# shunpeizhang/nebula

Measured on AMD Instinct MI355X. Metric: GO 3 STEPS traversed edges/sec (TEPS) at 1/2/4/8 GPU; FIND SHORTEST PATH p50, higher is better.
Workload: dtype int64; 1 GPU; GO 3 STEPS FROM <root> OVER e WHERE e.w < 50 YIELD e._dst, 16 single-root queries per step; graph=RMAT-26, parts=100, roots=16, queries_in_flight=6, parallelism=single, vertices_rank0=32799492, live_edges_out_plus_in_rank0=2120776948

## Files before the change

nebula_amd/csrc/final.hip:

```cpp
#include <hip/hip_runtime.h>

#include "nbg_internal.h"

namespace nbg {
namespace {

constexpr int FB = 256;
constexpr int FW = FB / 64;
constexpr int FV = VT;
static_assert(FV == 4 && TILE == 256, "the head mask is 4 words of 64 tile positions");

__device__ __forceinline__ void wave_lds_sync() {
  __builtin_amdgcn_fence(__ATOMIC_RELEASE, "wavefront");
  __builtin_amdgcn_wave_barrier();
  __builtin_amdgcn_fence(__ATOMIC_ACQUIRE, "wavefront");
}

template <typename T>
__device__ __forceinline__ T ld(const T* p) {
  return __hip_atomic_load(p, __ATOMIC_RELAXED, __HIP_MEMORY_SCOPE_WAVEFRONT);
}

template <int WB>
struct WType { using T = int64_t; };
template <> struct WType<1> { using T = int8_t; };
template <> struct WType<2> { using T = int16_t; };
template <> struct WType<4> { using T = int32_t; };

}

template <int WB, bool ONE>
__global__ void __launch_bounds__(FB) __attribute__((amdgpu_waves_per_eu(8)))
k_final_dst(FinalDstArgs a) {
  __shared__ unsigned long long sMaskAll[FW][FV];
  __shared__ uint32_t sDeltaAll[FW][TILE + 1];
  __shared__ unsigned long long sBase;
  const int lane = threadIdx.x & 63;
  const int w = __builtin_amdgcn_readfirstlane(threadIdx.x >> 6);
  unsigned long long* const sMask = sMaskAll[w];
  uint32_t* const sDelta = sDeltaAll[w];
  const uint64_t g = (uint64_t)gridDim.x * FW;
  uint64_t t = (uint64_t)blockIdx.x * FW + w;
  const __attribute__((address_space(4))) uint32_t* const tsplit =
      (const __attribute__((address_space(4))) uint32_t*)a.tsplit;
  const uint64_t tmax = a.tsplit_n ? a.tsplit_n - 1 : 0;
  auto clampt = [&](uint64_t x) { return x < tmax ? x : tmax; };
  const uint32_t sp0 = tsplit[clampt(t)], sp1 = tsplit[clampt(t + 1)];
  const uint32_t sq0 = tsplit[clampt(t + g)], sq1 = tsplit[clampt(t + g + 1)];
// ... 25 lines not shown
    *st = q == 0 ? 0u : (q - 1 < n32 ? x0 : 0xFFFFFFFFu);
    *en = q < n32 ? x1 : 0xFFFFFFFFu;
    *r = q < n32 ? rr : 0u;
  };
  const typename WType<WB>::T* const wcol = static_cast<const typename WType<WB>::T*>(a.wcol);
  int64_t wlo = a.lo, whi = a.hi;
  bool wneg = a.where_neg != 0;
  if (wlo < INT32_MIN) wlo = INT32_MIN;
  if (whi > INT32_MAX) whi = INT32_MAX;
  if (wlo > whi) {
    wlo = INT32_MIN;
    whi = INT32_MAX;
    wneg = !wneg;
  }
  const uint32_t wbase = (uint32_t)(int32_t)wlo, wspan = (uint32_t)(whi - wlo);
  auto store_rows = [&](const int64_t (&dv)[FV], uint32_t pm, uint64_t region) {
    uint32_t off = 0;
#pragma unroll
    for (int i = 0; i < FV; ++i) {
      const bool pass = (pm >> i) & 1u;
      const unsigned long long bal = __ballot(pass);
      const uint64_t row = region + off + __builtin_amdgcn_mbcnt_hi((uint32_t)(bal >> 32),
                                                                  __builtin_amdgcn_mbcnt_lo((uint32_t)bal, 0u));
      off += (uint32_t)__popcll(bal);
      if constexpr (ONE) {
        if (pass) a.out[0][row] = dv[i];
      } else {
        for (int y = 0; y < a.nyields; ++y)
          if (pass) a.out[y][row] = ((a.const_mask >> y) & 1u) ? a.yconst[y] : dv[i];
      }
    }
  };
  int64_t pdv[FV];
  uint32_t ppm = 0;
  uint64_t preg = 0;
#pragma unroll
  for (int i = 0; i < FV; ++i) pdv[i] = 0;
  uint64_t a0 = 0, a1 = 0, n0 = 0, n1 = 0;
  uint32_t e_pre = 0, f_pre = 0, r_pre = 0;
  if (t < ntiles) {
    a0 = sp0;
    a1 = (t + 1) * TILE >= npath ? n : sp1;
    if (t + g < ntiles) {
      n0 = sq0;
      n1 = (t + g + 1) * TILE >= npath ? n : sq1;
    }
    stage(a0, &e_pre, &f_pre, &r_pre);
  }
// ... 33 lines not shown
      }
    }
    wave_lds_sync();
    uint32_t jj[FV];
    {
      uint32_t before = 0;
#pragma unroll
      for (int i = 0; i < FV; ++i) {
        const unsigned long long m = sMask[i];
        const uint32_t c = before + (uint32_t)__popcll(m & le);
        before += (uint32_t)__popcll(m);
        jj[i] = b0 + (uint32_t)(i * 64 + lane) + sDelta[c];
      }
    }
    wave_lds_sync();
    int64_t dv[FV];
    typename WType<WB>::T x[FV];
    {
      const uint32_t jsafe = nb > 0 ? (uint32_t)__builtin_amdgcn_readfirstlane((int)jj[0]) : 0u;
#pragma unroll
      for (int i = 0; i < FV; ++i)
        if (i * 64 + lane >= nb) jj[i] = jsafe;
#pragma unroll
      for (int i = 0; i < FV; ++i) dv[i] = ld(a.dst_vid + jj[i]);
      if constexpr (WB != 0) {
#pragma unroll
        for (int i = 0; i < FV; ++i) x[i] = ld(wcol + jj[i]);
      }
    }
    store_rows(pdv, ppm, preg);
    uint32_t pm = 0;
#pragma unroll
    for (int i = 0; i < FV; ++i) {
      const bool act = i * 64 + lane < nb;
      bool pass = act;
      if constexpr (WB == 8) {
        const int64_t v = (int64_t)x[i];
        pass = act & (((v >= a.lo) & (v <= a.hi)) != (a.where_neg != 0));
      } else if constexpr (WB != 0) {
// ... 27 lines not shown
  }
  __syncthreads();
  if (threadIdx.x == 0) a.blk_rows[blockIdx.x] = (uint32_t)sBase;
}

namespace {

template <int WB>
void launch_wb(const FinalDstArgs& a, bool one, unsigned grid, hipStream_t s) {
  if (one) hipLaunchKernelGGL((k_final_dst<WB, true>), dim3(grid), dim3(FB), 0, s, a);
  else hipLaunchKernelGGL((k_final_dst<WB, false>), dim3(grid), dim3(FB), 0, s, a);
}

}

hipError_t launch_final_dst(const FinalDstArgs& a, int wbytes, bool one, unsigned grid, hipStream_t s) {
  switch (wbytes) {
    case 0: launch_wb<0>(a, one, grid, s); break;
    case 1: launch_wb<1>(a, one, grid, s); break;
    case 2: launch_wb<2>(a, one, grid, s); break;
    case 4: launch_wb<4>(a, one, grid, s); break;
    case 8: launch_wb<8>(a, one, grid, s); break;
    default: return hipErrorInvalidValue;
  }
  return hipGetLastError();
}

}
```

nebula_amd/csrc/finalcopy.hip:

```cpp
#include <hip/hip_runtime.h>

#include "nbg_internal.h"

namespace nbg {
namespace {

constexpr int CB = 256;
constexpr int CW = CB / 64;
constexpr int CH = 512;
constexpr int CM = CH / 64;
constexpr int CI = CH / 128;
static_assert(CH % 128 == 0, "a chunk is whole 16-byte stores of 64 lanes");

typedef long long row2 __attribute__((ext_vector_type(2), aligned(8)));

__device__ __forceinline__ void wave_lds_sync() {
  __builtin_amdgcn_fence(__ATOMIC_RELEASE, "wavefront");
  __builtin_amdgcn_wave_barrier();
  __builtin_amdgcn_fence(__ATOMIC_ACQUIRE, "wavefront");
}

template <typename T>
__device__ __forceinline__ T ld(const T* p) {
  return __hip_atomic_load(p, __ATOMIC_RELAXED, __HIP_MEMORY_SCOPE_WAVEFRONT);
}

__device__ __forceinline__ uint32_t lanes_below(unsigned long long b) {
  return __builtin_amdgcn_mbcnt_hi((uint32_t)(b >> 32), __builtin_amdgcn_mbcnt_lo((uint32_t)b, 0u));
}

}

__global__ void __launch_bounds__(CB) __attribute__((amdgpu_waves_per_eu(8)))
k_final_copy(FinalCopyArgs a) {
  __shared__ unsigned long long sMaskAll[CW][CM];
  __shared__ uint32_t sDeltaAll[CW][CH + 1];
  const int lane = threadIdx.x & 63;
  const int w = __builtin_amdgcn_readfirstlane(threadIdx.x >> 6);
  unsigned long long* const sMask = sMaskAll[w];
  uint32_t* const sDelta = sDeltaAll[w];
  const uint32_t g = gridDim.x * CW;
  const uint32_t t_first = blockIdx.x * CW + w;
  const unsigned long long packed = *a.acc;
  const uint64_t n = packed >> 32;
  const uint32_t n32 = (uint32_t)n, total = (uint32_t)packed;
  if (blockIdx.x == 0 && threadIdx.x == 0) {
    if (a.stat_e && !a.full_rp) *a.stat_e += total;
    if (a.stat_n) *a.stat_n = n;
  }
// ... 86 lines not shown
      idx[2 * i] = r0 + p + sDelta[base + (uint32_t)__popcll(m & le0)];
      idx[2 * i + 1] = r0 + p + 1 + sDelta[base + (uint32_t)__popcll(m & le1)];
      before += c0 + (uint32_t)__popcll(m1);
    }
    wave_lds_sync();
    const uint32_t jsafe = ok ? (uint32_t)__builtin_amdgcn_readfirstlane((int)idx[0]) : 0u;
#pragma unroll
    for (int i = 0; i < CI; ++i) {
      const uint32_t p = (uint32_t)(i * 128 + 2 * lane);
      if (!ok || p >= nb) idx[2 * i] = jsafe;
      if (!ok || p + 1 >= nb) idx[2 * i + 1] = jsafe;
    }
    return ok;
  };
  auto store2 = [&](int64_t* p, row2 v) { __builtin_nontemporal_store(v, reinterpret_cast<row2*>(p)); };
  auto store_chunk = [&](const row2 (&v)[CI], uint32_t tt) {
    int64_t* const o = out + (uint64_t)tt * CH + 2 * lane;
#pragma unroll
    for (int i = 0; i < CI; ++i) store2(o + i * 128, v[i]);
  };
  auto fetch = [&](uint32_t tt, uint32_t kb, uint32_t x0, uint32_t x1, uint32_t rr, row2 (&v)[CI]) {
    const uint32_t r0 = tt * CH;
    uint32_t st, en, rs;
    window(kb, x0, x1, rr, &st, &en, &rs);
    const unsigned long long own = __ballot(kb + (uint32_t)lane < n32 && st <= r0 && r0 < en);
    const int l0 = own ? __ffsll((long long)own) - 1 : 0;
    const uint32_t st0 = (uint32_t)__builtin_amdgcn_readlane((int)st, l0);
    const uint32_t en0 = (uint32_t)__builtin_amdgcn_readlane((int)en, l0);
    const uint32_t rs0 = (uint32_t)__builtin_amdgcn_readlane((int)rs, l0);
    if (own && en0 - r0 >= (uint32_t)CH) {
      const int64_t* const src = a.dst_vid + (uint64_t)(rs0 + (r0 - st0)) + 2 * lane;
#pragma unroll
      for (int i = 0; i < CI; ++i) v[i] = *reinterpret_cast<const row2*>(src + i * 128);
    } else {
      uint32_t idx[2 * CI];
      const bool ok = resolve(kb, r0, CH, st, en, rs, idx);
      if (!ok && lane == 0) atomicOr(a.err_flag, SPLIT_BAD);
#pragma unroll
      for (int i = 0; i < CI; ++i) {
        v[i].x = ld(a.dst_vid + idx[2 * i]);
        v[i].y = ld(a.dst_vid + idx[2 * i + 1]);
      }
    }
  };
  const uint32_t mine = t_first < nfull ? (nfull - 1 - t_first) / g + 1 : 0u;
  uint32_t a_lo = 0, a_hi = 0, a_step = 0, a_val = 0, b_lo = 0, b_hi = 0, b_step = 0, b_val = 0;
  bool a_pend = false, b_pend = false;
  uint32_t s_kb = 0, s_x0 = 0, s_x1 = 0, s_rr = 0;
  row2 cur[CI];
#pragma unroll
  for (int i = 0; i < CI; ++i) cur[i] = row2{0, 0};
  for (uint32_t it = 0; mine && it < mine + 4; ++it) {
    if (it >= 4) store_chunk(cur, t_first + (it - 4) * g);
    if (it >= 3 && it < mine + 3) fetch(t_first + (it - 3) * g, s_kb, s_x0, s_x1, s_rr, cur);
    if (it >= 2 && it < mine + 2) {
      if (b_pend) narrow(&b_lo, &b_hi, b_step, b_val, (t_first + (it - 2) * g) * CH);
      s_kb = b_lo;
      stage(s_kb, &s_x0, &s_x1, &s_rr);
    }
    if (it >= 1 && it < mine + 1) {
      b_lo = a_lo;
      b_hi = a_hi;
      if (a_pend) narrow(&b_lo, &b_hi, a_step, a_val, (t_first + (it - 1) * g) * CH);
      b_pend = b_hi - b_lo > 64;
      if (b_pend) {
        b_step = (b_hi - b_lo + 63) / 64;
// ... 6 lines not shown
      if (a_pend) {
        a_step = (a_hi - a_lo + 63) / 64;
        a_val = probe(a_lo, a_hi, a_step);
      }
    }
  }
  const uint32_t rem = total - nfull * CH;
  if (rem && t_first == nfull % g) {
    const uint32_t r0 = nfull * CH;
    const uint32_t kb = bracket(r0);
    uint32_t x0, x1, rr, st, en, rs, idx[2 * CI];
    stage(kb, &x0, &x1, &rr);
    window(kb, x0, x1, rr, &st, &en, &rs);
    const bool ok = resolve(kb, r0, rem, st, en, rs, idx);
    if (!ok && lane == 0) atomicOr(a.err_flag, SPLIT_BAD);
    int64_t v[2 * CI];
#pragma unroll
    for (int i = 0; i < 2 * CI; ++i) v[i] = ld(a.dst_vid + idx[i]);
#pragma unroll
    for (int i = 0; i < CI; ++i) {
      const uint32_t p = (uint32_t)(i * 128 + 2 * lane);
      if (ok && p < rem) out[(uint64_t)r0 + p] = v[2 * i];
      if (ok && p + 1 < rem) out[(uint64_t)r0 + p + 1] = v[2 * i + 1];
    }
  }
  if (a.full_rp) {
    unsigned long long sum = 0;
    for (uint64_t i = (uint64_t)t_first * 64 + lane; i < n; i += (uint64_t)g * 64) {
      const uint32_t v = a.ids[i];
      if (v != NO_ROW && (!a.visible || a.visible[v])) sum += a.full_rp[v + 1] - a.full_rp[v];
    }
    for (int o = 32; o; o >>= 1) sum += __shfl_down(sum, o, 64);
    if (lane == 0 && sum) atomicAdd(a.stat_e, sum);
  }
  if (threadIdx.x == 0) a.blk_rows[blockIdx.x] = blockIdx.x == 0 ? total : 0u;
}

hipError_t launch_final_copy(const FinalCopyArgs& a, unsigned grid, hipStream_t s) {
  hipLaunchKernelGGL(k_final_copy, dim3(grid), dim3(CB), 0, s, a);
  return hipGetLastError();
}

}
```

nebula_amd/csrc/go.cpp:

```cpp
#include <algorithm>
#include <array>
#include <atomic>
#include <cstring>
#include <ctime>
#include <iterator>
#include <set>
#include <unordered_map>

#include "engine.h"
#include "nbg_rows.h"

using namespace nbg;

struct nbg_go_stmt {
  Engine* eng = nullptr;
  uint64_t id = 0;
  std::vector<int32_t> over;
  std::vector<TypeProgram> plist;
  int ncols = 0;
  uint32_t steps = 1;
  int32_t deferred = NBG_OK;
  std::string deferred_msg;
  std::string dst_unknown;
  bool distinct = false;
// ... 1 lines not shown
  std::vector<std::vector<uint8_t>> wclass;
  bool misaligned = false, float_col = false;
  bool derived = false;
  uint64_t sout_row_bytes = 0;
  bool uses_input = false;
  std::vector<int64_t> in_ids;
  std::vector<std::vector<int64_t>> in_cols;
  uint64_t in_n = 0;
  int64_t* d_in_ids = nullptr;
  int64_t** d_in_cols = nullptr;
  std::vector<int64_t*> d_in_col_ptrs;
  std::vector<std::string> in_xstr;
  uint32_t* d_xoff = nullptr;
  char* d_xbytes = nullptr;
  bool idx_on = false;
  double idx_after = 0.25;
  uint64_t idx_budget = UINT64_MAX;
  uint64_t final_scanned = 0;
  StmtIndex idx;
  bool idx_tried = false;
  void free_input_index() {
    for (void* p : {(void*)d_in_ids, (void*)d_in_cols, (void*)d_xoff, (void*)d_xbytes})
      if (p) (void)hipFree(p);
    for (auto* p : d_in_col_ptrs)
      if (p) (void)hipFree(p);
    d_in_ids = nullptr;
    d_in_cols = nullptr;
    d_xoff = nullptr;
    d_xbytes = nullptr;
    d_in_col_ptrs.clear();
// ... 505 lines not shown
  Engine& E = q.E;
  nbg_go_stmt* st = q.st;
  if (!st->idx_on || st->idx_tried || st->steps < 2 || E.partitioned() || st->deferred || st->over.empty()) return;
  auto it = E.snap.types.find(st->over[0]);
  if (it == E.snap.types.end()) return;
  const DevEdgeType& dt = it->second;
  if ((double)st->final_scanned < st->idx_after * (double)dt.num_edges) return;
  st->idx_tried = true;
  if ((uint64_t)q.cap < (uint64_t)std::max(dt.max_degree, 0)) return;
  const TypeProgram& prog = st->plist[0];
  if (prog.where_const) return;
  StmtIndexSpec sp{};
  if (!ws_final_where(prog, q.args_for(dt), &sp)) return;
  sp.nv = E.snap.nv;
  sp.edges = dt.num_edges;
  double ms = 0;
  const bool ok = stmtidx_build(sp, st->idx_budget, E.stream, &st->idx, &ms);
  if (getenv("NBG_STMT_INDEX_TRACE")) {
    if (ok)
      fprintf(stderr, "[stmt index] statement %llu type %d: built in %.3f ms after %llu final-step edges, %llu of %llu "
                      "edges pass, %.1f MB\n", (unsigned long long)st->id, st->over[0], ms,
              (unsigned long long)st->final_scanned, (unsigned long long)st->idx.rows,
              (unsigned long long)dt.num_edges, (double)st->idx.bytes / 1e6);
    else
      fprintf(stderr, "[stmt index] statement %llu type %d: not built (memory budget or allocation), %.3f ms\n",
              (unsigned long long)st->id, st->over[0], ms);
  }
}

static void go_workspace(GoQuery& q, const GoStarts& S, uint64_t num_starts, Workspace** wsp) {
  Engine& E = q.E;
  if (!q.lrc && *wsp) {
    const int32_t rrc = ws_release(E, wsp, q.stream);
    if (rrc) q.local_fail(rrc, E.last_error);
  }
  const uint64_t need = q.part ? std::max<uint64_t>(num_starts, 1) : S.n;
  const uint64_t e_need = std::max<uint64_t>(E.snap.max_edges(), S.start_edges);
  if (!q.lrc && (!*wsp || need > ws_cap_frontier(*wsp) || S.n + S.start_edges > ws_cap_items(*wsp))) {
// ... 152 lines not shown
      }
    }
    if (s == 1 && !final && hop1_slots) he = ws_set_hop_slots(ws, hop1_slots);
    for (size_t i = 0; he == hipSuccess && i < over.size(); ++i) {
      auto it = E.snap.types.find(over[i]);
      if (it == E.snap.types.end()) continue;
      ExpandArgs a = q.args_for(it->second);
      a.bt_first = s == 1;
      if (!final) {
        he = ws_expand_mark(ws, a, n_bound, it->second.num_edges, (int)s, (int)i, S.inline_of(i, s), np0);
      } else if (q.st->deferred || (plist[i].where_const && !plist[i].where_const_val)) {
        he = ws_scan_only(ws, a, n_bound, (int)s, (int)i);
      } else if (const StmtIndex* ix = q.index_of(i)) {
        const uint32_t* const full = a.row_ptr;
        a.row_ptr = ix->rp;
        a.dst_vid = ix->dst;
        he = ws_expand_final(ws, a, n_bound, ebound[i], (int)s, (int)i, plist[i], plan.region[i], plan.blk_cap[i],
                             nullptr, full);
      } else {
        he = ws_expand_final(ws, a, n_bound, ebound[i], (int)s, (int)i, plist[i], plan.region[i], plan.blk_cap[i],
                             S.inline_of(i, s));
      }
    }
    if (inject) he = hipErrorLaunchFailure;
    if (!final && he == hipSuccess) {
      he = q.part ? ws_exchange(ws, (int)s, np0) : ws_finish_step(ws, (int)s, np0);
      n_bound = E.snap.nv;
    }
  }
  return he;
}

static hipError_t go_end(const GoQuery& q, const RowPlan& plan, bool device) {
// ... 555 lines not shown
  for (int32_t i = 0; i < cap && i < (int32_t)req.size(); ++i) out[i] = req[i];
  return (int32_t)req.size();
}

int32_t nbg_go_prepare(nbg_engine* h, const nbg_go_request* req, nbg_go_stmt** out) {
  if (!h) return NBG_E_INVALID_ARGUMENT;
  Engine& E = h->e;
  std::lock_guard<std::mutex> lg(E.mu);
  const int32_t rc = go_prepare(E, req, out);
  if (rc || (*out)->steps < 2) return rc;
  {
    nbg_go_stmt* st = *out;
    const char* on = getenv("NBG_STMT_INDEX");
    const char* after = getenv("NBG_STMT_INDEX_AFTER");
    const char* mb = getenv("NBG_STMT_INDEX_MB");
    st->idx_on = !(on && atoi(on) == 0);
    if (after) st->idx_after = std::max(0.0, atof(after));
    if (mb) st->idx_budget = strtoull(mb, nullptr, 10) << 20;
  }
  if (hipSetDevice(E.cfg.device) != hipSuccess) return NBG_OK;
  const uint64_t rows = stmt_row_bound(E, *out);
  auto reserve = [&](Workspace* w) {
    if (w && !E.holders.count(w)) (void)ws_reserve_rows(w, rows, (*out)->ncols);
  };
  reserve(E.ws);
  for (auto& q : E.slots) reserve(q.ws);
  E.row_reserve = std::max(E.row_reserve, rows);
  E.col_reserve = std::max(E.col_reserve, (*out)->ncols);
  return NBG_OK;
}

// ... 16 lines not shown
```

nebula_amd/csrc/kernels.hip:

```cpp
#include <hip/hip_runtime.h>
#include <array>
#include <cstddef>

#include <cstdio>
#include <cstring>
#include <vector>

#include "aggops.h"
#include "stage.h"
#include "ws.h"

namespace nbg {


struct DegSrc {
  const uint32_t* row_ptr;
  const uint8_t* visible;
  uint32_t cap;
};

struct ListOut {
  uint32_t* ids;
  uint32_t* seg_end;
  uint32_t* seg_rs;
// ... 2175 lines not shown
    unsigned long long e = 0;
    for (int t = 0; t < ntypes; ++t) e += q->e_st[s][t];
    g[1 + (MAX_STEPS + 2) + s] = e;
  }
}

static double prof_bytes(const Workspace* w, const Prof::Rec& r, const QState& q) {
  switch (r.kid) {
    case K_RELIST: return 12.0 * (double)q.step_n[r.step];
    case K_EXPAND_MARK: return 4.0 * (double)q.e_st[r.step][r.tix];
    case K_COMPACT: case K_BITS_COMPACT: return 16.0 * (double)q.step_n[r.step + 1];
    case K_PACK: case K_ALLTOALL: case K_ROOTS: return r.cols;
    case K_EXPAND_FINAL: {
      double rows = 0;
      for (unsigned b = 0; b < w->final_grid[r.tix]; ++b) rows += (double)w->h_blk_rows[(size_t)r.tix * EXPAND_GRID + b];
      if (r.cols < 0) return 8.0 * rows + 8.0 * rows * r.kout + 12.0 * (double)q.step_n[r.step];
      return (double)q.e_st[r.step][r.tix] * (4.0 + 8.0 * r.cols) + 8.0 * rows * r.kout;
    }
    default: return 0.0;
  }
}
static double prof_bytes_path(const Prof::Rec& r, const PState& p) {
  const int i = r.step < PATH_REC ? r.step : PATH_REC - 1;
  switch (r.kid) {
    case K_RELIST: return 12.0 * (double)p.ln[i];
    case K_BFS: return 4.0 * (double)p.le[i];
    case K_GATHER: return 8.0 * (double)p.lc[i];
    case K_DEGSUM: return 12.0 * (double)p.ln[i];
    default: return 0.0;
  }
}
// ... 566 lines not shown
  if (prog.yield_reg.size() > (size_t)MAX_YIELDS) return false;
  const FastProg f = detect_fast(prog, a);
  if (!final_where_shape(f, a)) return false;
  sp->row_ptr = a.row_ptr;
  sp->dst_vid = a.dst_vid;
  sp->wcol = f.wcol;
  sp->wbytes = f.wbytes;
  sp->lo = f.lo;
  sp->hi = f.hi;
  sp->where_neg = f.where_neg;
  return true;
}

hipError_t ws_expand_final(Workspace* w, const ExpandArgs& a0, uint64_t n_bound, uint64_t e_bound, int step, int tix,
                           const TypeProgram& prog, uint64_t region_base, uint64_t blk_cap, const InlineList* il,
                           const uint32_t* full_row_ptr) {
  if (step > MAX_STEPS || tix >= MAX_TYPES_Q) return hipErrorInvalidValue;
  const bool inl = inline_start_list(w, tix, il);
  if (full_row_ptr && (inl || tix != 0 || !w->seg_ready)) return hipErrorInvalidValue;
  const ListRef L = inl ? ListRef{nullptr, nullptr, &w->q->step_n[step], 0} : prepare_list(w, a0, n_bound, step, tix);
  ExpandArgs a = a0;
  a.frontier = L.ids;
  a.tsplit = inl ? nullptr : set_split(w, L.set);
  uint32_t* const l_end = set_end(w, L.set);
  uint32_t* const l_rs = set_rs(w, L.set);
  FinalParams fp{};
  fp.prog = w->d_prog + (size_t)tix * MAX_PROGRAM;
  fp.where_len = prog.where_len;
  fp.where_reg = prog.where_reg;
  fp.prog_len = (int)prog.code.size();
  fp.nyields = (int)prog.yield_reg.size();
  for (int y = 0; y < fp.nyields; ++y) {
// ... 63 lines not shown
    if (full_row_ptr && one && final_copy_on()) {
      FinalCopyArgs ca{};
      ca.acc = fa.acc;
      ca.seg_end = fa.seg_end;
      ca.seg_rs = fa.seg_rs;
      ca.dst_vid = fa.dst_vid;
      ca.out = fa.out[0];
      ca.region_base = region_base;
      ca.blk_rows = fa.blk_rows;
      ca.stat_e = fa.stat_e;
      ca.stat_n = fa.stat_n;
      ca.err_flag = fa.err_flag;
      ca.full_rp = fa.full_rp;
      ca.ids = fa.ids;
      ca.visible = fa.visible;
      le = launch_final_copy(ca, grid.x, w->stream);
    } else {
      le = launch_final_dst(fa, fp.fast.has_where ? fp.fast.wbytes : 0, one, grid.x, w->stream);
    }
    if (le != hipSuccess) {
      prof_end(w, p, K_EXPAND_FINAL, step, tix, 0.0, 0.0);
      return le;
    }
  } else {
    launch(grid, lds, w->stream, a, L.acc, l_end, l_rs, w->flags, fp, BfsParams{}, e_st, L.stat_n, inl ? il : nullptr);
  }
  prof_end(w, p, K_EXPAND_FINAL, step, tix, full_row_ptr ? -1.0 : (double)edge_columns_read(prog), (double)fp.nyields);
  w->final_grid[tix] = final_grid(n_bound, e_bound);
  return hipGetLastError();
}



hipError_t ws_backtracker(Workspace* w, int64_t** out, int64_t** in) {
  if (!w->bt) HIP_TRY(hipMalloc((void**)&w->bt, (w->nv + 1) * 8));
  if (w->comm && !w->h_btc) {
    const uint64_t G = (uint64_t)w->comm->world, nwords = G * w->npad / 64;
    if (!w->bt_out) HIP_TRY(hipMalloc((void**)&w->bt_out, G * w->npad * 8));
    if (!w->bt_pack) HIP_TRY(hipMalloc((void**)&w->bt_pack, G * w->npad * 8));
    if (!w->bt_recv) HIP_TRY(hipMalloc((void**)&w->bt_recv, G * w->npad * 8));
    if (!w->bt_pre) HIP_TRY(hipMalloc((void**)&w->bt_pre, 2 * nwords * 4));
    if (!w->bt_boff) HIP_TRY(hipMalloc((void**)&w->bt_boff, 2 * (nwords / RW_BLOCK) * 4));
// ... 1583 lines not shown
```

nebula_amd/csrc/nbg_internal.h:

```cpp
#pragma once
#include <hip/hip_runtime_api.h>

#include <array>
#include <cstdint>
#include <map>
#include <memory>
#include <string>
#include <unordered_map>
#include <vector>

#include "../../include/nbg.h"

namespace nbg {

constexpr uint32_t NO_ROW = 0xFFFFFFFFu;

struct Column {
  std::string name;
  int32_t type;
};
struct Schema {
  int64_t version = 0;
  std::vector<Column> cols;
  int find(const std::string& n) const {
// ... 287 lines not shown
  uint64_t in_n;
  const int64_t* const* in_cols;
  DevStrings str;
  int64_t now_sec;
  uint64_t rand_seed;
};

struct FinalDstArgs {
  const unsigned long long* acc;
  const uint32_t* seg_end;
  const uint32_t* seg_rs;
  const uint32_t* tsplit;
  uint64_t tsplit_n;
  const int64_t* dst_vid;
  const void* wcol;
  int64_t lo, hi;
  int32_t where_neg;
  int32_t nyields;
  uint64_t const_mask;
  int64_t yconst[MAX_YIELDS];
  int64_t* out[MAX_YIELDS];
  uint64_t region_base, blk_cap;
  uint32_t* blk_rows;
  unsigned long long* stat_e;
  unsigned long long* stat_n;
  unsigned long long* err_flag;
  const uint32_t* full_rp;
  const uint32_t* ids;
  const uint8_t* visible;
};
hipError_t launch_final_dst(const FinalDstArgs& a, int wbytes, bool one, unsigned grid, hipStream_t s);

struct FinalCopyArgs {
  const unsigned long long* acc;
  const uint32_t* seg_end;
  const uint32_t* seg_rs;
  const int64_t* dst_vid;
  int64_t* out;
  uint64_t region_base;
  uint32_t* blk_rows;
  unsigned long long* stat_e;
  unsigned long long* stat_n;
  unsigned long long* err_flag;
  const uint32_t* full_rp;
  const uint32_t* ids;
  const uint8_t* visible;
};
hipError_t launch_final_copy(const FinalCopyArgs& a, unsigned grid, hipStream_t s);

struct StmtIndexSpec {
  const uint32_t* row_ptr;
  const int64_t* dst_vid;
  uint64_t nv, edges;
  const void* wcol;
  int wbytes;
  int64_t lo, hi;
  int where_neg;
};
struct StmtIndex {
  uint32_t* rp = nullptr;
  int64_t* dst = nullptr;
  uint64_t rows = 0;
  uint64_t bytes = 0;
};
bool stmtidx_build(const StmtIndexSpec& sp, uint64_t budget_bytes, hipStream_t s, StmtIndex* out, double* ms);
void stmtidx_free(StmtIndex* ix);

constexpr int LVL_BITS = 6;
constexpr uint32_t MAX_PATH_LEN = (1u << LVL_BITS) - 1;
constexpr int PSLOTS = 8;
enum PathLabel { LAB_F = 0, LAB_B = 1, LAB_S = 2, LAB_M = 3, NUM_LABS = 4 };
constexpr int GREEDY_HOP_BLOCKS = 64;
constexpr int PATH_REC = 64;

struct PState {
  unsigned long long n[PSLOTS];
  unsigned long long total;
  unsigned long long edges;
// ... 524 lines not shown
uint64_t rd_block_bytes(uint64_t len, uint64_t nchunks, uint64_t rows);
int32_t ws_rows_decode(hipStream_t stream, const uint8_t* data, uint64_t len, const uint64_t* chunk_start, uint64_t nchunks,
                       const uint32_t* row_off, uint64_t rows, void* block, const RdPlan& plan, Workspace** outw,
                       RdRecord* rec, StageProf<RD_KINDS>* prof, std::string* err);

hipError_t ws_begin_query(Workspace* w, const uint32_t* starts, uint64_t n, const std::vector<TypeProgram>* progs,
                          uint64_t stmt_id);
hipError_t ws_begin_query_resident(Workspace* w, uint64_t n, const std::vector<TypeProgram>* progs, uint64_t stmt_id);
hipError_t ws_expand_mark(Workspace* w, const ExpandArgs& a, uint64_t n_bound, uint64_t e_bound, int step, int tix,
                          const InlineList* il, const ExpandArgs* next0);
hipError_t ws_finish_step(Workspace* w, int step, const ExpandArgs* next0);
void ws_set_mark_claims(Workspace* w, bool claims);
void ws_set_wake(Workspace* w, bool flag);
hipError_t ws_expand_final(Workspace* w, const ExpandArgs& a, uint64_t n_bound, uint64_t e_bound, int step, int tix,
                           const TypeProgram& prog, uint64_t region_base, uint64_t blk_cap, const InlineList* il = nullptr,
                           const uint32_t* full_row_ptr = nullptr);
bool ws_final_where(const TypeProgram& prog, const ExpandArgs& a, StmtIndexSpec* sp);
hipError_t ws_scan_only(Workspace* w, const ExpandArgs& a, uint64_t n_bound, int step, int tix);
hipError_t ws_backtracker(Workspace* w, int64_t** out, int64_t** in);
void ws_backtracker_off(Workspace* w);
hipError_t ws_end_query(Workspace* w);
hipError_t ws_end_query_async(Workspace* w);
struct SmallPack {
  int ntypes, ncols;
  uint64_t region[MAX_TYPES_Q], blk_cap[MAX_TYPES_Q];
  uint32_t grid[MAX_TYPES_Q];
};
constexpr uint64_t SMALL_ROWS_WORDS = 32768;
hipError_t ws_end_query_async_small(Workspace* w, const SmallPack& sp);
const int64_t* ws_host_small_rows(Workspace* w, uint64_t count);
hipError_t ws_end_query_wait(Workspace* w);
// ... 90 lines not shown
```

nebula_amd/csrc/stmtidx.hip:

```cpp
#include <hip/hip_runtime.h>

#include <algorithm>
#include <chrono>
#include <cstring>
#include <rocprim/rocprim.hpp>

#include "nbg_internal.h"

namespace nbg {
namespace {

constexpr int BT = 256;

unsigned grid_for(uint64_t n) {
  const uint64_t g = (n + BT - 1) / BT;
  return (unsigned)std::min<uint64_t>(std::max<uint64_t>(g, 1), 1u << 16);
}

#define GRID_STRIDE(i, n) \
  for (uint64_t i = (uint64_t)blockIdx.x * BT + threadIdx.x; i < (n); i += (uint64_t)gridDim.x * BT)

template <typename T>
struct Pass {
  const T* col;
  int64_t lo, hi;
  bool neg;
  uint64_t n;
  __device__ __forceinline__ uint32_t operator()(uint64_t j) const {
    if (j >= n) return 0u;
    const int64_t v = (int64_t)col[j];
    return (((v >= lo) & (v <= hi)) != neg) ? 1u : 0u;
  }
};

template <typename T>
__global__ void __launch_bounds__(BT) k_idx_scatter(Pass<T> pass, const uint32_t* __restrict__ pos,
                                                    const int64_t* __restrict__ dst, int64_t* __restrict__ out) {
  GRID_STRIDE(j, pass.n)
    if (pass(j)) out[pos[j]] = dst[j];
}

__global__ void __launch_bounds__(BT) k_idx_rows(const uint32_t* __restrict__ row_ptr, const uint32_t* __restrict__ pos,
                                                 uint32_t* __restrict__ rp, uint64_t nv) {
  GRID_STRIDE(v, nv + 1) rp[v] = pos[row_ptr[v]];
}

struct Temps {
  uint32_t* pos = nullptr;
  void* scan = nullptr;
  ~Temps() {
    if (pos) (void)hipFree(pos);
    if (scan) (void)hipFree(scan);
  }
};

template <typename T>
bool build_as(const StmtIndexSpec& sp, uint64_t budget, hipStream_t s, StmtIndex* out) {
  const uint64_t E = sp.edges, nv = sp.nv;
  const Pass<T> pass{static_cast<const T*>(sp.wcol), sp.lo, sp.hi, sp.where_neg != 0, E};
  auto flags = rocprim::make_transform_iterator(rocprim::make_counting_iterator<uint64_t>(0), pass);
  size_t scan_bytes = 0;
  Temps t;
  if (rocprim::exclusive_scan(nullptr, scan_bytes, flags, t.pos, 0u, E + 1, rocprim::plus<uint32_t>(), s) != hipSuccess)
    return false;
  const uint64_t rp_bytes = (nv + 1) * 4, temp_bytes = (E + 1) * 4 + scan_bytes;
  if (rp_bytes + temp_bytes > budget) return false;
  StmtIndex ix;
  bool ok = hipMalloc((void**)&t.pos, (E + 1) * 4) == hipSuccess &&
            hipMalloc(&t.scan, std::max<size_t>(scan_bytes, 1)) == hipSuccess &&
            hipMalloc((void**)&ix.rp, rp_bytes) == hipSuccess;
  ok = ok && rocprim::exclusive_scan(t.scan, scan_bytes, flags, t.pos, 0u, E + 1, rocprim::plus<uint32_t>(), s) ==
                 hipSuccess;
  uint32_t total = 0;
  ok = ok && hipMemcpyAsync(&total, t.pos + E, 4, hipMemcpyDeviceToHost, s) == hipSuccess &&
       hipStreamSynchronize(s) == hipSuccess;
  const uint64_t dst_bytes = std::max<uint64_t>(total, 1) * 8;
  ok = ok && rp_bytes + dst_bytes + temp_bytes <= budget && hipMalloc((void**)&ix.dst, dst_bytes) == hipSuccess;
  if (ok) {
    if (!total) ok = hipMemsetAsync(ix.dst, 0, 8, s) == hipSuccess;
    hipLaunchKernelGGL(k_idx_rows, dim3(grid_for(nv + 1)), dim3(BT), 0, s, sp.row_ptr, t.pos, ix.rp, nv);
    if (total) hipLaunchKernelGGL(k_idx_scatter<T>, dim3(grid_for(E)), dim3(BT), 0, s, pass, t.pos, sp.dst_vid, ix.dst);
    ok = ok && hipGetLastError() == hipSuccess && hipStreamSynchronize(s) == hipSuccess;
  }
  if (!ok) {
    (void)hipGetLastError();
    stmtidx_free(&ix);
    return false;
  }
  ix.rows = total;
  ix.bytes = rp_bytes + dst_bytes;
  *out = ix;
  return true;
}

}

void stmtidx_free(StmtIndex* ix) {
  if (ix->rp) (void)hipFree(ix->rp);
  if (ix->dst) (void)hipFree(ix->dst);
  *ix = StmtIndex{};
}

bool stmtidx_build(const StmtIndexSpec& sp, uint64_t budget_bytes, hipStream_t s, StmtIndex* out, double* ms) {
  *out = StmtIndex{};
  if (!sp.row_ptr || !sp.dst_vid || !sp.wcol || !sp.edges || sp.edges >= 0xFFFFFFFFull) return false;
  size_t free_b = 0, total_b = 0;
  if (hipMemGetInfo(&free_b, &total_b) != hipSuccess) return false;
  const uint64_t budget = std::min<uint64_t>(budget_bytes, free_b / 2);
  if (hipStreamSynchronize(s) != hipSuccess) return false;
  const auto t0 = std::chrono::steady_clock::now();
  bool ok = false;
  switch (sp.wbytes) {
    case 1: ok = build_as<int8_t>(sp, budget, s, out); break;
    case 2: ok = build_as<int16_t>(sp, budget, s, out); break;
    case 4: ok = build_as<int32_t>(sp, budget, s, out); break;
    case 8: ok = build_as<int64_t>(sp, budget, s, out); break;
    default: break;
  }
  if (ms) *ms = std::chrono::duration<double, std::milli>(std::chrono::steady_clock::now() - t0).count();
  return ok;
}

}
```

Measured before the change: 591.1 billion TEPS.

## Store statement-index destination IDs as 32-bit offsets from a base

When building the per-statement filtered edge index, a reduction first finds the min/max destination vertex ID. If the span fits in 32 bits, destinations are stored as uint32 offsets from that base. The final-step dst and copy kernels read the narrower column and widen it back to int64 on output. This halves the bytes read from the index in the final GO step, at the cost of an extra reduction pass during index build and more kernel template variants.

```diff
diff --git a/nebula_amd/csrc/final.hip b/nebula_amd/csrc/final.hip
--- a/nebula_amd/csrc/final.hip
+++ b/nebula_amd/csrc/final.hip
@@ -27,11 +27,22 @@
 template <> struct WType<2> { using T = int16_t; };
 template <> struct WType<4> { using T = int32_t; };
 
-}
-
-template <int WB, bool ONE>
+constexpr int DST32 = -4;
+template <int WB>
+struct DType { using T = int64_t; };
+template <> struct DType<DST32> { using T = uint32_t; };
+
+}
+
+template <int WBX, bool ONE>
 __global__ void __launch_bounds__(FB) __attribute__((amdgpu_waves_per_eu(8)))
 k_final_dst(FinalDstArgs a) {
+  constexpr int WB = WBX == DST32 ? 0 : WBX;
+  using DT = typename DType<WBX>::T;
+  auto wide = [&](DT c) -> int64_t {
+    if constexpr (WBX == DST32) return (int64_t)((uint64_t)a.dst_base + (uint64_t)c);
+    else return c;
+  };
   __shared__ unsigned long long sMaskAll[FW][FV];
   __shared__ uint32_t sDeltaAll[FW][TILE + 1];
   __shared__ unsigned long long sBase;
@@ -87,7 +98,7 @@
     wneg = !wneg;
   }
   const uint32_t wbase = (uint32_t)(int32_t)wlo, wspan = (uint32_t)(whi - wlo);
-  auto store_rows = [&](const int64_t (&dv)[FV], uint32_t pm, uint64_t region) {
+  auto store_rows = [&](const DT (&dv)[FV], uint32_t pm, uint64_t region) {
     uint32_t off = 0;
 #pragma unroll
     for (int i = 0; i < FV; ++i) {
@@ -97,14 +108,14 @@
                                                                   __builtin_amdgcn_mbcnt_lo((uint32_t)bal, 0u));
       off += (uint32_t)__popcll(bal);
       if constexpr (ONE) {
-        if (pass) a.out[0][row] = dv[i];
+        if (pass) a.out[0][row] = wide(dv[i]);
       } else {
         for (int y = 0; y < a.nyields; ++y)
-          if (pass) a.out[y][row] = ((a.const_mask >> y) & 1u) ? a.yconst[y] : dv[i];
-      }
-    }
-  };
-  int64_t pdv[FV];
+          if (pass) a.out[y][row] = ((a.const_mask >> y) & 1u) ? a.yconst[y] : wide(dv[i]);
+      }
+    }
+  };
+  DT pdv[FV];
   uint32_t ppm = 0;
   uint64_t preg = 0;
 #pragma unroll
@@ -168,7 +179,7 @@
       }
     }
     wave_lds_sync();
-    int64_t dv[FV];
+    DT dv[FV];
     typename WType<WB>::T x[FV];
     {
       const uint32_t jsafe = nb > 0 ? (uint32_t)__builtin_amdgcn_readfirstlane((int)jj[0]) : 0u;
@@ -176,7 +187,7 @@
       for (int i = 0; i < FV; ++i)
         if (i * 64 + lane >= nb) jj[i] = jsafe;
 #pragma unroll
-      for (int i = 0; i < FV; ++i) dv[i] = ld(a.dst_vid + jj[i]);
+      for (int i = 0; i < FV; ++i) dv[i] = ld(reinterpret_cast<const DT*>(a.dst_vid) + jj[i]);
       if constexpr (WB != 0) {
 #pragma unroll
         for (int i = 0; i < FV; ++i) x[i] = ld(wcol + jj[i]);
@@ -234,7 +245,12 @@
 
 }
 
-hipError_t launch_final_dst(const FinalDstArgs& a, int wbytes, bool one, unsigned grid, hipStream_t s) {
+hipError_t launch_final_dst(const FinalDstArgs& a, int wbytes, bool one, bool dst32, unsigned grid, hipStream_t s) {
+  if (dst32) {
+    if (wbytes != 0) return hipErrorInvalidValue;
+    launch_wb<DST32>(a, one, grid, s);
+    return hipGetLastError();
+  }
   switch (wbytes) {
     case 0: launch_wb<0>(a, one, grid, s); break;
     case 1: launch_wb<1>(a, one, grid, s); break;
diff --git a/nebula_amd/csrc/finalcopy.hip b/nebula_amd/csrc/finalcopy.hip
--- a/nebula_amd/csrc/finalcopy.hip
+++ b/nebula_amd/csrc/finalcopy.hip
@@ -13,6 +13,21 @@
 static_assert(CH % 128 == 0, "a chunk is whole 16-byte stores of 64 lanes");
 
 typedef long long row2 __attribute__((ext_vector_type(2), aligned(8)));
+typedef unsigned long long cell2 __attribute__((aligned(4)));
+static_assert(__alignof__(row2) == 8 && __alignof__(cell2) == 4, "a run starts at any element");
+
+template <int DB>
+struct Src {
+  typedef int64_t one;
+  typedef row2 two;
+};
+template <>
+struct Src<4> {
+  typedef uint32_t one;
+  typedef cell2 two;
+};
+
+}
 
 __device__ __forceinline__ void wave_lds_sync() {
   __builtin_amdgcn_fence(__ATOMIC_RELEASE, "wavefront");
@@ -29,10 +44,20 @@
   return __builtin_amdgcn_mbcnt_hi((uint32_t)(b >> 32), __builtin_amdgcn_mbcnt_lo((uint32_t)b, 0u));
 }
 
-}
-
+template <int DB>
 __global__ void __launch_bounds__(CB) __attribute__((amdgpu_waves_per_eu(8)))
-k_final_copy(FinalCopyArgs a) {
+k_final_copy(FinalCopyArgs a, int64_t base) {
+  using one = typename Src<DB>::one;
+  using two = typename Src<DB>::two;
+  const one* const dst = reinterpret_cast<const one*>(a.dst_vid);
+  auto wide1 = [&](one c) -> int64_t {
+    if constexpr (DB == 4) return (int64_t)((uint64_t)base + (uint64_t)c);
+    else return c;
+  };
+  auto wide2 = [&](two c) -> row2 {
+    if constexpr (DB == 4) return row2{(long long)wide1((uint32_t)c), (long long)wide1((uint32_t)(c >> 32))};
+    else return c;
+  };
   __shared__ unsigned long long sMaskAll[CW][CM];
   __shared__ uint32_t sDeltaAll[CW][CH + 1];
   const int lane = threadIdx.x & 63;
@@ -149,12 +174,12 @@
     return ok;
   };
   auto store2 = [&](int64_t* p, row2 v) { __builtin_nontemporal_store(v, reinterpret_cast<row2*>(p)); };
-  auto store_chunk = [&](const row2 (&v)[CI], uint32_t tt) {
+  auto store_chunk = [&](const two (&v)[CI], uint32_t tt) {
     int64_t* const o = out + (uint64_t)tt * CH + 2 * lane;
 #pragma unroll
-    for (int i = 0; i < CI; ++i) store2(o + i * 128, v[i]);
-  };
-  auto fetch = [&](uint32_t tt, uint32_t kb, uint32_t x0, uint32_t x1, uint32_t rr, row2 (&v)[CI]) {
+    for (int i = 0; i < CI; ++i) store2(o + i * 128, wide2(v[i]));
+  };
+  auto fetch = [&](uint32_t tt, uint32_t kb, uint32_t x0, uint32_t x1, uint32_t rr, two (&v)[CI]) {
     const uint32_t r0 = tt * CH;
     uint32_t st, en, rs;
     window(kb, x0, x1, rr, &st, &en, &rs);
@@ -164,17 +189,18 @@
     const uint32_t en0 = (uint32_t)__builtin_amdgcn_readlane((int)en, l0);
     const uint32_t rs0 = (uint32_t)__builtin_amdgcn_readlane((int)rs, l0);
     if (own && en0 - r0 >= (uint32_t)CH) {
-      const int64_t* const src = a.dst_vid + (uint64_t)(rs0 + (r0 - st0)) + 2 * lane;
-#pragma unroll
-      for (int i = 0; i < CI; ++i) v[i] = *reinterpret_cast<const row2*>(src + i * 128);
+      const one* const src = dst + (uint64_t)(rs0 + (r0 - st0)) + 2 * lane;
+#pragma unroll
+      for (int i = 0; i < CI; ++i) v[i] = *reinterpret_cast<const two*>(src + i * 128);
     } else {
       uint32_t idx[2 * CI];
       const bool ok = resolve(kb, r0, CH, st, en, rs, idx);
       if (!ok && lane == 0) atomicOr(a.err_flag, SPLIT_BAD);
 #pragma unroll
       for (int i = 0; i < CI; ++i) {
-        v[i].x = ld(a.dst_vid + idx[2 * i]);
-        v[i].y = ld(a.dst_vid + idx[2 * i + 1]);
+        const one x = ld(dst + idx[2 * i]), y = ld(dst + idx[2 * i + 1]);
+        if constexpr (DB == 4) v[i] = (unsigned long long)x | (unsigned long long)y << 32;
+        else v[i] = row2{x, y};
       }
     }
   };
@@ -182,9 +208,9 @@
   uint32_t a_lo = 0, a_hi = 0, a_step = 0, a_val = 0, b_lo = 0, b_hi = 0, b_step = 0, b_val = 0;
   bool a_pend = false, b_pend = false;
   uint32_t s_kb = 0, s_x0 = 0, s_x1 = 0, s_rr = 0;
-  row2 cur[CI];
-#pragma unroll
-  for (int i = 0; i < CI; ++i) cur[i] = row2{0, 0};
+  two cur[CI];
+#pragma unroll
+  for (int i = 0; i < CI; ++i) cur[i] = two{};
   for (uint32_t it = 0; mine && it < mine + 4; ++it) {
     if (it >= 4) store_chunk(cur, t_first + (it - 4) * g);
     if (it >= 3 && it < mine + 3) fetch(t_first + (it - 3) * g, s_kb, s_x0, s_x1, s_rr, cur);
@@ -221,14 +247,14 @@
     window(kb, x0, x1, rr, &st, &en, &rs);
     const bool ok = resolve(kb, r0, rem, st, en, rs, idx);
     if (!ok && lane == 0) atomicOr(a.err_flag, SPLIT_BAD);
-    int64_t v[2 * CI];
-#pragma unroll
-    for (int i = 0; i < 2 * CI; ++i) v[i] = ld(a.dst_vid + idx[i]);
+    one v[2 * CI];
+#pragma unroll
+    for (int i = 0; i < 2 * CI; ++i) v[i] = ld(dst + idx[i]);
 #pragma unroll
     for (int i = 0; i < CI; ++i) {
       const uint32_t p = (uint32_t)(i * 128 + 2 * lane);
-      if (ok && p < rem) out[(uint64_t)r0 + p] = v[2 * i];
-      if (ok && p + 1 < rem) out[(uint64_t)r0 + p + 1] = v[2 * i + 1];
+      if (ok && p < rem) out[(uint64_t)r0 + p] = wide1(v[2 * i]);
+      if (ok && p + 1 < rem) out[(uint64_t)r0 + p + 1] = wide1(v[2 * i + 1]);
     }
   }
   if (a.full_rp) {
@@ -243,8 +269,9 @@
   if (threadIdx.x == 0) a.blk_rows[blockIdx.x] = blockIdx.x == 0 ? total : 0u;
 }
 
-hipError_t launch_final_copy(const FinalCopyArgs& a, unsigned grid, hipStream_t s) {
-  hipLaunchKernelGGL(k_final_copy, dim3(grid), dim3(CB), 0, s, a);
+hipError_t launch_final_copy(const FinalCopyArgs& a, bool dst32, int64_t dst_base, unsigned grid, hipStream_t s) {
+  if (dst32) hipLaunchKernelGGL(k_final_copy<4>, dim3(grid), dim3(CB), 0, s, a, dst_base);
+  else hipLaunchKernelGGL(k_final_copy<8>, dim3(grid), dim3(CB), 0, s, a, (int64_t)0);
   return hipGetLastError();
 }
 
diff --git a/nebula_amd/csrc/go.cpp b/nebula_amd/csrc/go.cpp
--- a/nebula_amd/csrc/go.cpp
+++ b/nebula_amd/csrc/go.cpp
@@ -39,6 +39,7 @@
   uint32_t* d_xoff = nullptr;
   char* d_xbytes = nullptr;
   bool idx_on = false;
+  bool idx_dst32 = true;
   double idx_after = 0.25;
   uint64_t idx_budget = UINT64_MAX;
   uint64_t final_scanned = 0;
@@ -574,14 +575,16 @@
   if (!ws_final_where(prog, q.args_for(dt), &sp)) return;
   sp.nv = E.snap.nv;
   sp.edges = dt.num_edges;
+  sp.dst32 = st->idx_dst32 ? 1 : 0;
   double ms = 0;
   const bool ok = stmtidx_build(sp, st->idx_budget, E.stream, &st->idx, &ms);
   if (getenv("NBG_STMT_INDEX_TRACE")) {
     if (ok)
-      fprintf(stderr, "[stmt index] statement %llu type %d: built in %.3f ms after %llu final-step edges, %llu of %llu "
-                      "edges pass, %.1f MB\n", (unsigned long long)st->id, st->over[0], ms,
-              (unsigned long long)st->final_scanned, (unsigned long long)st->idx.rows,
-              (unsigned long long)dt.num_edges, (double)st->idx.bytes / 1e6);
+      fprintf(stderr, "[stmt index] statement %llu type %d: built in %.3f ms (_dst range pass %.3f ms) after %llu "
+                      "final-step edges, %llu of %llu edges pass, %.1f MB, %d-byte _dst, base %lld\n",
+              (unsigned long long)st->id, st->over[0], ms, st->idx.range_ms, (unsigned long long)st->final_scanned,
+              (unsigned long long)st->idx.rows, (unsigned long long)dt.num_edges, (double)st->idx.bytes / 1e6,
+              st->idx.dst_bytes, (long long)st->idx.base);
     else
       fprintf(stderr, "[stmt index] statement %llu type %d: not built (memory budget or allocation), %.3f ms\n",
               (unsigned long long)st->id, st->over[0], ms);
@@ -764,9 +767,9 @@
       } else if (const StmtIndex* ix = q.index_of(i)) {
         const uint32_t* const full = a.row_ptr;
         a.row_ptr = ix->rp;
-        a.dst_vid = ix->dst;
+        a.dst_vid = static_cast<const int64_t*>(ix->dst);
         he = ws_expand_final(ws, a, n_bound, ebound[i], (int)s, (int)i, plist[i], plan.region[i], plan.blk_cap[i],
-                             nullptr, full);
+                             nullptr, full, ix->dst_bytes, ix->base);
       } else {
         he = ws_expand_final(ws, a, n_bound, ebound[i], (int)s, (int)i, plist[i], plan.region[i], plan.blk_cap[i],
                              S.inline_of(i, s));
@@ -1352,7 +1355,9 @@
     const char* on = getenv("NBG_STMT_INDEX");
     const char* after = getenv("NBG_STMT_INDEX_AFTER");
     const char* mb = getenv("NBG_STMT_INDEX_MB");
+    const char* d32 = getenv("NBG_STMT_INDEX_DST32");
     st->idx_on = !(on && atoi(on) == 0);
+    st->idx_dst32 = !(d32 && atoi(d32) == 0);
     if (after) st->idx_after = std::max(0.0, atof(after));
     if (mb) st->idx_budget = strtoull(mb, nullptr, 10) << 20;
   }
diff --git a/nebula_amd/csrc/kernels.hip b/nebula_amd/csrc/kernels.hip
--- a/nebula_amd/csrc/kernels.hip
+++ b/nebula_amd/csrc/kernels.hip
@@ -2213,7 +2213,7 @@
     case K_EXPAND_FINAL: {
       double rows = 0;
       for (unsigned b = 0; b < w->final_grid[r.tix]; ++b) rows += (double)w->h_blk_rows[(size_t)r.tix * EXPAND_GRID + b];
-      if (r.cols < 0) return 8.0 * rows + 8.0 * rows * r.kout + 12.0 * (double)q.step_n[r.step];
+      if (r.cols < 0) return -r.cols * rows + 8.0 * rows * r.kout + 12.0 * (double)q.step_n[r.step];
       return (double)q.e_st[r.step][r.tix] * (4.0 + 8.0 * r.cols) + 8.0 * rows * r.kout;
     }
     default: return 0.0;
@@ -2810,8 +2810,10 @@
 
 hipError_t ws_expand_final(Workspace* w, const ExpandArgs& a0, uint64_t n_bound, uint64_t e_bound, int step, int tix,
                            const TypeProgram& prog, uint64_t region_base, uint64_t blk_cap, const InlineList* il,
-                           const uint32_t* full_row_ptr) {
+                           const uint32_t* full_row_ptr, int dst_bytes, int64_t dst_base) {
   if (step > MAX_STEPS || tix >= MAX_TYPES_Q) return hipErrorInvalidValue;
+  if (full_row_ptr ? dst_bytes != 8 && dst_bytes != 4 : dst_bytes != 8) return hipErrorInvalidValue;
+  const bool dst32 = dst_bytes == 4;
   const bool inl = inline_start_list(w, tix, il);
   if (full_row_ptr && (inl || tix != 0 || !w->seg_ready)) return hipErrorInvalidValue;
   const ListRef L = inl ? ListRef{nullptr, nullptr, &w->q->step_n[step], 0} : prepare_list(w, a0, n_bound, step, tix);
@@ -2905,18 +2907,24 @@
       ca.full_rp = fa.full_rp;
       ca.ids = fa.ids;
       ca.visible = fa.visible;
-      le = launch_final_copy(ca, grid.x, w->stream);
+      le = launch_final_copy(ca, dst32, dst_base, grid.x, w->stream);
     } else {
-      le = launch_final_dst(fa, fp.fast.has_where ? fp.fast.wbytes : 0, one, grid.x, w->stream);
+      if (dst32) fa.dst_base = dst_base;
+      le = launch_final_dst(fa, fp.fast.has_where ? fp.fast.wbytes : 0, one, dst32, grid.x, w->stream);
     }
     if (le != hipSuccess) {
       prof_end(w, p, K_EXPAND_FINAL, step, tix, 0.0, 0.0);
       return le;
     }
   } else {
+    if (dst32) {
+      prof_end(w, p, K_EXPAND_FINAL, step, tix, 0.0, 0.0);
+      return hipErrorInvalidValue;
+    }
     launch(grid, lds, w->stream, a, L.acc, l_end, l_rs, w->flags, fp, BfsParams{}, e_st, L.stat_n, inl ? il : nullptr);
   }
-  prof_end(w, p, K_EXPAND_FINAL, step, tix, full_row_ptr ? -1.0 : (double)edge_columns_read(prog), (double)fp.nyields);
+  prof_end(w, p, K_EXPAND_FINAL, step, tix, full_row_ptr ? -(double)dst_bytes : (double)edge_columns_read(prog),
+           (double)fp.nyields);
   w->final_grid[tix] = final_grid(n_bound, e_bound);
   return hipGetLastError();
 }
diff --git a/nebula_amd/csrc/nbg_internal.h b/nebula_amd/csrc/nbg_internal.h
--- a/nebula_amd/csrc/nbg_internal.h
+++ b/nebula_amd/csrc/nbg_internal.h
@@ -325,7 +325,11 @@
   uint64_t tsplit_n;
   const int64_t* dst_vid;
   const void* wcol;
-  int64_t lo, hi;
+  union {
+    int64_t lo;
+    int64_t dst_base;
+  };
+  int64_t hi;
   int32_t where_neg;
   int32_t nyields;
   uint64_t const_mask;
@@ -340,7 +344,7 @@
   const uint32_t* ids;
   const uint8_t* visible;
 };
-hipError_t launch_final_dst(const FinalDstArgs& a, int wbytes, bool one, unsigned grid, hipStream_t s);
+hipError_t launch_final_dst(const FinalDstArgs& a, int wbytes, bool one, bool dst32, unsigned grid, hipStream_t s);
 
 struct FinalCopyArgs {
   const unsigned long long* acc;
@@ -357,7 +361,7 @@
   const uint32_t* ids;
   const uint8_t* visible;
 };
-hipError_t launch_final_copy(const FinalCopyArgs& a, unsigned grid, hipStream_t s);
+hipError_t launch_final_copy(const FinalCopyArgs& a, bool dst32, int64_t dst_base, unsigned grid, hipStream_t s);
 
 struct StmtIndexSpec {
   const uint32_t* row_ptr;
@@ -367,12 +371,16 @@
   int wbytes;
   int64_t lo, hi;
   int where_neg;
+  int dst32;
 };
 struct StmtIndex {
   uint32_t* rp = nullptr;
-  int64_t* dst = nullptr;
+  void* dst = nullptr;
+  int dst_bytes = 8;
+  int64_t base = 0;
   uint64_t rows = 0;
   uint64_t bytes = 0;
+  double range_ms = 0;
 };
 bool stmtidx_build(const StmtIndexSpec& sp, uint64_t budget_bytes, hipStream_t s, StmtIndex* out, double* ms);
 void stmtidx_free(StmtIndex* ix);
@@ -927,7 +935,7 @@
 void ws_set_wake(Workspace* w, bool flag);
 hipError_t ws_expand_final(Workspace* w, const ExpandArgs& a, uint64_t n_bound, uint64_t e_bound, int step, int tix,
                            const TypeProgram& prog, uint64_t region_base, uint64_t blk_cap, const InlineList* il = nullptr,
-                           const uint32_t* full_row_ptr = nullptr);
+                           const uint32_t* full_row_ptr = nullptr, int dst_bytes = 8, int64_t dst_base = 0);
 bool ws_final_where(const TypeProgram& prog, const ExpandArgs& a, StmtIndexSpec* sp);
 hipError_t ws_scan_only(Workspace* w, const ExpandArgs& a, uint64_t n_bound, int step, int tix);
 hipError_t ws_backtracker(Workspace* w, int64_t** out, int64_t** in);
diff --git a/nebula_amd/csrc/stmtidx.hip b/nebula_amd/csrc/stmtidx.hip
--- a/nebula_amd/csrc/stmtidx.hip
+++ b/nebula_amd/csrc/stmtidx.hip
@@ -33,11 +33,46 @@
   }
 };
 
-template <typename T>
+template <typename T, typename D>
 __global__ void __launch_bounds__(BT) k_idx_scatter(Pass<T> pass, const uint32_t* __restrict__ pos,
-                                                    const int64_t* __restrict__ dst, int64_t* __restrict__ out) {
+                                                    const int64_t* __restrict__ dst, D* __restrict__ out, int64_t base) {
   GRID_STRIDE(j, pass.n)
-    if (pass(j)) out[pos[j]] = dst[j];
+    if (pass(j)) out[pos[j]] = (D)((uint64_t)dst[j] - (uint64_t)base);
+}
+
+struct Range {
+  int64_t lo, hi;
+};
+struct RangeOf {
+  const int64_t* dst;
+  __device__ __forceinline__ Range operator()(uint64_t j) const {
+    const int64_t v = dst[j];
+    return Range{v, v};
+  }
+};
+struct RangeJoin {
+  __device__ __forceinline__ Range operator()(const Range& a, const Range& b) const {
+    return Range{a.lo < b.lo ? a.lo : b.lo, a.hi > b.hi ? a.hi : b.hi};
+  }
+};
+
+bool dst_range(const int64_t* dst, uint64_t E, hipStream_t s, Range* out) {
+  (void)hipGetLastError();
+  auto vals = rocprim::make_transform_iterator(rocprim::make_counting_iterator<uint64_t>(0), RangeOf{dst});
+  const Range init{INT64_MAX, INT64_MIN};
+  size_t bytes = 0;
+  Range* d_out = nullptr;
+  void* tmp = nullptr;
+  bool ok = rocprim::reduce(nullptr, bytes, vals, d_out, init, E, RangeJoin(), s) == hipSuccess &&
+            hipMalloc((void**)&d_out, sizeof(Range)) == hipSuccess &&
+            hipMalloc(&tmp, std::max<size_t>(bytes, 1)) == hipSuccess &&
+            rocprim::reduce(tmp, bytes, vals, d_out, init, E, RangeJoin(), s) == hipSuccess &&
+            hipMemcpyAsync(out, d_out, sizeof(Range), hipMemcpyDeviceToHost, s) == hipSuccess &&
+            hipStreamSynchronize(s) == hipSuccess;
+  if (d_out) (void)hipFree(d_out);
+  if (tmp) (void)hipFree(tmp);
+  if (!ok) (void)hipGetLastError();
+  return ok;
 }
 
 __global__ void __launch_bounds__(BT) k_idx_rows(const uint32_t* __restrict__ row_ptr, const uint32_t* __restrict__ pos,
@@ -55,7 +90,7 @@
 };
 
 template <typename T>
-bool build_as(const StmtIndexSpec& sp, uint64_t budget, hipStream_t s, StmtIndex* out) {
+bool build_as(const StmtIndexSpec& sp, uint64_t budget, hipStream_t s, int dst_bytes, int64_t base, StmtIndex* out) {
   const uint64_t E = sp.edges, nv = sp.nv;
   const Pass<T> pass{static_cast<const T*>(sp.wcol), sp.lo, sp.hi, sp.where_neg != 0, E};
   auto flags = rocprim::make_transform_iterator(rocprim::make_counting_iterator<uint64_t>(0), pass);
@@ -74,12 +109,18 @@
   uint32_t total = 0;
   ok = ok && hipMemcpyAsync(&total, t.pos + E, 4, hipMemcpyDeviceToHost, s) == hipSuccess &&
        hipStreamSynchronize(s) == hipSuccess;
-  const uint64_t dst_bytes = std::max<uint64_t>(total, 1) * 8;
-  ok = ok && rp_bytes + dst_bytes + temp_bytes <= budget && hipMalloc((void**)&ix.dst, dst_bytes) == hipSuccess;
+  const uint64_t col_bytes = std::max<uint64_t>(total, 1) * (uint64_t)dst_bytes;
+  ok = ok && rp_bytes + col_bytes + temp_bytes <= budget &&
+       hipMalloc(&ix.dst, std::max<uint64_t>(col_bytes, 8)) == hipSuccess;
   if (ok) {
-    if (!total) ok = hipMemsetAsync(ix.dst, 0, 8, s) == hipSuccess;
+    if (total < 2) ok = hipMemsetAsync(ix.dst, 0, 8, s) == hipSuccess;
     hipLaunchKernelGGL(k_idx_rows, dim3(grid_for(nv + 1)), dim3(BT), 0, s, sp.row_ptr, t.pos, ix.rp, nv);
-    if (total) hipLaunchKernelGGL(k_idx_scatter<T>, dim3(grid_for(E)), dim3(BT), 0, s, pass, t.pos, sp.dst_vid, ix.dst);
+    if (total && dst_bytes == 4)
+      hipLaunchKernelGGL((k_idx_scatter<T, uint32_t>), dim3(grid_for(E)), dim3(BT), 0, s, pass, t.pos, sp.dst_vid,
+                         static_cast<uint32_t*>(ix.dst), base);
+    else if (total)
+      hipLaunchKernelGGL((k_idx_scatter<T, int64_t>), dim3(grid_for(E)), dim3(BT), 0, s, pass, t.pos, sp.dst_vid,
+                         static_cast<int64_t*>(ix.dst), (int64_t)0);
     ok = ok && hipGetLastError() == hipSuccess && hipStreamSynchronize(s) == hipSuccess;
   }
   if (!ok) {
@@ -88,7 +129,9 @@
     return false;
   }
   ix.rows = total;
-  ix.bytes = rp_bytes + dst_bytes;
+  ix.dst_bytes = dst_bytes;
+  ix.base = dst_bytes == 4 ? base : 0;
+  ix.bytes = rp_bytes + col_bytes;
   *out = ix;
   return true;
 }
@@ -109,15 +152,25 @@
   const uint64_t budget = std::min<uint64_t>(budget_bytes, free_b / 2);
   if (hipStreamSynchronize(s) != hipSuccess) return false;
   const auto t0 = std::chrono::steady_clock::now();
+  auto since = [&] { return std::chrono::duration<double, std::milli>(std::chrono::steady_clock::now() - t0).count(); };
+  int dst_bytes = 8;
+  Range r{0, 0};
+  double range_ms = 0;
+  if (sp.dst32) {
+    const bool known = dst_range(sp.dst_vid, sp.edges, s, &r) && r.lo <= r.hi;
+    if (known && (uint64_t)r.hi - (uint64_t)r.lo < (1ull << 32)) dst_bytes = 4;
+    range_ms = known ? since() : -1.0;
+  }
   bool ok = false;
   switch (sp.wbytes) {
-    case 1: ok = build_as<int8_t>(sp, budget, s, out); break;
-    case 2: ok = build_as<int16_t>(sp, budget, s, out); break;
-    case 4: ok = build_as<int32_t>(sp, budget, s, out); break;
-    case 8: ok = build_as<int64_t>(sp, budget, s, out); break;
+    case 1: ok = build_as<int8_t>(sp, budget, s, dst_bytes, r.lo, out); break;
+    case 2: ok = build_as<int16_t>(sp, budget, s, dst_bytes, r.lo, out); break;
+    case 4: ok = build_as<int32_t>(sp, budget, s, dst_bytes, r.lo, out); break;
+    case 8: ok = build_as<int64_t>(sp, budget, s, dst_bytes, r.lo, out); break;
     default: break;
   }
-  if (ms) *ms = std::chrono::duration<double, std::milli>(std::chrono::steady_clock::now() - t0).count();
+  if (ok) out->range_ms = range_ms;
+  if (ms) *ms = since();
   return ok;
 }
 
```

Result: slower. 581.6 billion TEPS (-1.6%).
